# Fable3/CarND-Path-Planning-Project

Hardware: NVIDIA B200
Metric: planned frames/sec at 1M-frame batch (higher is better)
Workload: dtype f64

## Files before the change

### carnd-path-planning-project_b200/__init__.py

```python
from __future__ import annotations

import ctypes as C
import os

os.environ.setdefault("CUDA_DEVICE_MAX_CONNECTIONS", "32")

import numpy as np

from . import abi
from .abi import (Config, FrameBatch, Frames, PlanBatch, Plans, default_config, FLAG, FLAG_NAMES,
                  NUM_FLAGS, STATS_LEN, PATH_LEN, PREV_KEEP, MAP_STRIDE, FSTATS_LEN, FSTAT_NMIN,
                  FSTAT_NAMES, COMM_ID_BYTES)

_HERE = os.path.dirname(os.path.abspath(__file__))
LIB_PATH = os.path.join(_HERE, "libpp_b200.so")
ROOT = os.path.dirname(_HERE)
MAP_CSV = os.path.join(ROOT, "data", "highway_map.csv")

EXPORTS = [
    "pp_version", "pp_init", "pp_strerror", "pp_last_cuda_error", "pp_device_count", "pp_config_default",
    "pp_map_create", "pp_map_create_from_csv", "pp_map_destroy", "pp_map_num_waypoints",
    "pp_map_table", "pp_plan_batch", "pp_plan_batch_host", "pp_plan_batch_host_split", "pp_stats_batch",
    "pp_set_kernel_variant", "pp_launch_count", "pp_distancesq_pt_seg_batch",
    "pp_init_reference_waypoint_batch", "pp_lane_matching_batch", "pp_get_lane_pos_batch",
    "pp_spline_batch", "pp_closest_waypoint_batch", "pp_next_waypoint_batch",
    "pp_get_frenet_batch", "pp_get_xy_batch", "pp_synth_frames", "pp_selftest_math",
    "pp_lane_change_batch", "pp_limit_speed_batch", "pp_trajectory_build_batch",
    "pp_set_phase_timing", "pp_get_phase_ms", "pp_speed_controller_batch",
    "pp_project_speed_batch", "pp_control_points_batch",
    "pp_dev_alloc", "pp_dev_free", "pp_host_alloc", "pp_host_free", "pp_dev_upload", "pp_dev_download", "pp_dev_sync",
    "pp_dev_set", "pp_stream_create", "pp_stream_sync", "pp_stream_destroy",
    "pp_rollouts_create", "pp_rollouts_destroy", "pp_rollouts_run", "pp_rollouts_last",
    "pp_rollouts_get_state", "pp_rollouts_stats", "pp_rollouts_set_lean", "pp_rollouts_set_groups",
    "pp_rollouts_get_incidents", "pp_rollouts_incident_totals", "pp_rollouts_set_traffic",
    "pp_rollouts_get_traffic", "pp_rollouts_set_recorder", "pp_rollouts_get_recording",
    "pp_rollouts_set_surrogate", "pp_rollouts_get_surrogate", "pp_rollouts_surrogate_totals",
    "pp_sweep_batch",
    "pp_set_pipes", "pp_plan_stats_batch", "pp_synth_frames_dev", "pp_fstats_batch",
    "pp_comm_unique_id", "pp_comm_init_rank", "pp_comm_init_all", "pp_comm_destroy",
    "pp_comm_group_begin", "pp_comm_group_end", "pp_stats_reduce",
]


class PPError(RuntimeError):
    pass
# ... 511 lines not shown
```

### carnd-path-planning-project_b200/csrc/pp_api.cu

```cuda
#include <cuda_runtime.h>

#include <atomic>
#include <cstdint>
#include <cstdio>
#include <cstdlib>
#include <cstring>
#include <mutex>
#include <string>
#include <vector>

#include "pp_internal.h"

extern "C" int pp_init(void) {
  if (setenv("CUDA_DEVICE_MAX_CONNECTIONS", "32", 0) != 0) return PP_E_ARG;
  return PP_OK;
}

namespace {
std::mutex g_err_mu;
std::string g_err = "";
std::atomic<long long> g_launches{0};
}

namespace ppi {
// ... 11 lines not shown
int check_map_device(const pp_map *map, const char *who) {
  if (!map) return PP_E_ARG;
  if (!map->dev_table) {
    set_cuda_error(who, 0, "map has no device table (no usable CUDA device)");
    return PP_E_CUDA;
  }
  int dev = -1;
  cudaError_t e = cudaGetDevice(&dev);
  if (e != cudaSuccess) {
    set_cuda_error("cudaGetDevice", (int)e, cudaGetErrorString(e));
    cudaGetLastError();
    return PP_E_CUDA;
  }
  if (dev != map->device) {
    char msg[160];
    std::snprintf(msg, sizeof msg, "map lives on device %d but device %d is current", map->device,
                  dev);
    set_cuda_error(who, 0, msg);
    return PP_E_ARG;
  }
  return PP_OK;
}

int upload_map(pp_map *m) {
  int dev = 0;
  cudaError_t e = cudaGetDevice(&dev);
  if (e != cudaSuccess) {
    set_cuda_error("cudaGetDevice", (int)e, cudaGetErrorString(e));
    cudaGetLastError();
    return PP_E_CUDA;
  }
  const int pad = 24;
  static_assert(pad == PPD_PAD_ROWS, "padding must match the device code");
  std::vector<double> padded((size_t)(m->n + 2 * pad) * PP_MAP_STRIDE);
  for (int r = 0; r < m->n + 2 * pad; r++) {
    int src = (r - pad) % m->n;
    if (src < 0) src += m->n;
    std::memcpy(&padded[(size_t)r * PP_MAP_STRIDE], &m->table[(size_t)src * PP_MAP_STRIDE],
                PP_MAP_STRIDE * sizeof(double));
  }
  padded.resize(padded.size() + 2, 0.0);
  const size_t bytes = padded.size() * sizeof(double);
  e = cudaMalloc(&m->dev_table, bytes);
  if (e != cudaSuccess) {
    m->dev_table = nullptr;
    set_cuda_error("cudaMalloc(map)", (int)e, cudaGetErrorString(e));
    cudaGetLastError();
    return PP_E_CUDA;
  }
  e = cudaMemcpy(m->dev_table, padded.data(), bytes, cudaMemcpyHostToDevice);
  if (e != cudaSuccess) {
    cudaFree(m->dev_table);
    m->dev_table = nullptr;
    set_cuda_error("cudaMemcpy(map)", (int)e, cudaGetErrorString(e));
    cudaGetLastError();
    return PP_E_CUDA;
  }
  e = cudaMalloc(&m->dev_yaw, m->yaw.size() * sizeof(double));
  if (e == cudaSuccess)
    e = cudaMemcpy(m->dev_yaw, m->yaw.data(), m->yaw.size() * sizeof(double), cudaMemcpyHostToDevice);
  if (e != cudaSuccess) {
    cudaFree(m->dev_table);
// ... 91 lines not shown

int pp_map_create_from_csv(const char *path, pp_map **out) {
  if (!out) return PP_E_ARG;
  *out = nullptr;
  std::vector<double> wx, wy;
  int rc = ppi::read_map_csv(path, wx, wy);
  if (rc != PP_OK) return rc;
  return pp_map_create(wx.data(), wy.data(), (int)wx.size(), out);
}

void pp_map_destroy(pp_map *map) {
  if (!map) return;
  ppi::free_map_device(map);
  delete map;
}

int pp_map_num_waypoints(const pp_map *map) { return map ? map->n : PP_E_ARG; }

int pp_map_has_device(const pp_map *map) { return map && map->dev_table ? 1 : 0; }

int pp_map_table(const pp_map *map, double *out) {
  if (!map || !out) return PP_E_ARG;
  std::memcpy(out, map->table.data(), map->table.size() * sizeof(double));
  return PP_OK;
}

#define PP_CK(call, what)                                           \
  do {                                                              \
    cudaError_t e_ = (call);                                        \
    if (e_ != cudaSuccess) {                                        \
      ppi::set_cuda_error(what, (int)e_, cudaGetErrorString(e_));   \
      cudaGetLastError();                                           \
      return PP_E_CUDA;                                             \
    }                                                               \
  } while (0)

int pp_dev_alloc(void **out, size_t bytes) {
  if (!out) return PP_E_ARG;
  *out = nullptr;
  PP_CK(cudaMalloc(out, bytes ? bytes : 1), "pp_dev_alloc");
  return PP_OK;
}
int pp_dev_free(void *p) {
  if (p) PP_CK(cudaFree(p), "pp_dev_free");
  return PP_OK;
}
// ... 487 lines not shown
```

### carnd-path-planning-project_b200/csrc/pp_device.cuh

```cuda
#pragma once
#include <cstdint>

#include "../../include/pp.h"

namespace ppd {

#define PPD_EPS 1e-5
#define PPD_PI 3.14159265358979323846

#define PPD_INLINE __device__ __forceinline__

#define PPD_PAD 24
struct MapView {
  const double *t;
  int n;
  int pad_lo;
};

static __device__ __noinline__ int wrap_index(int idx, int n) {
  if (idx >= 0) return idx % n;
  idx += n;
  if (idx >= 0) return idx;
  unsigned long long k = (unsigned long long)(long long)idx;
  return (int)(k % (unsigned long long)n);
}

PPD_INLINE const double *row(const MapView &m, int idx) {
  if ((unsigned)(idx + m.pad_lo) < (unsigned)(m.n + m.pad_lo + PPD_PAD))
    return m.t + idx * PP_MAP_STRIDE;
  return m.t + wrap_index(idx, m.n) * PP_MAP_STRIDE;
}

__host__ __device__ inline size_t map_smem_doubles(int n) { return (size_t)(n + 2 * PPD_PAD) * PP_MAP_STRIDE; }

__host__ __device__ inline size_t map_stage_bytes(int n) {
  return (map_smem_doubles(n) * sizeof(double) + 15) & ~(size_t)15;
}

PPD_INLINE unsigned smem_addr(const void *p) { return (unsigned)__cvta_generic_to_shared(p); }
PPD_INLINE void mbar_init(unsigned bar, int count) {
  asm volatile("mbarrier.init.shared::cta.b64 [%0], %1;" ::"r"(bar), "r"(count) : "memory");
  asm volatile("fence.mbarrier_init.release.cluster;" ::: "memory");
}
PPD_INLINE void mbar_expect_tx(unsigned bar, unsigned bytes) {
  asm volatile("mbarrier.arrive.expect_tx.shared::cta.b64 _, [%0], %1;" ::"r"(bar), "r"(bytes)
               : "memory");
}
PPD_INLINE bool mbar_try_wait(unsigned bar, unsigned parity) {
  unsigned ok;
  asm volatile(
      "{\n"
      ".reg .pred p;\n"
      "mbarrier.try_wait.parity.shared::cta.b64 p, [%1], %2;\n"
      "selp.u32 %0, 1, 0, p;\n"
      "}\n"
      : "=r"(ok)
// ... 36 lines not shown
    asm volatile("mbarrier.init.shared::cta.b64 [%0], %1;" ::"r"(bar), "r"(1) : "memory");
    asm volatile("fence.mbarrier_init.release.cluster;" ::: "memory");
  }
  __syncthreads();
  if (threadIdx.x == 0) {
    asm volatile("mbarrier.arrive.expect_tx.shared::cta.b64 _, [%0], %1;" ::"r"(bar), "r"(bytes)
                 : "memory");
    asm volatile(
        "cp.async.bulk.shared::cluster.global.mbarrier::complete_tx::bytes [%0], [%1], %2, [%3];"
        ::"r"(dst), "l"(table), "r"(bytes), "r"(bar)
        : "memory");
  }
  asm volatile(
      "{\n"
      ".reg .pred p;\n"
      "WAIT_MAP:\n"
      "mbarrier.try_wait.parity.shared::cta.b64 p, [%0], %1;\n"
      "@p bra DONE_MAP;\n"
      "bra WAIT_MAP;\n"
      "DONE_MAP:\n"
      "}\n" ::"r"(bar), "r"(0)
      : "memory");
  MapView m;
  m.t = s_map + PPD_PAD * PP_MAP_STRIDE;
  m.n = n;
  m.pad_lo = n < PPD_PAD ? n : PPD_PAD;
  return m;
}

PPD_INLINE double vlen(double x, double y) { return sqrt(x * x + y * y); }
PPD_INLINE double dist4(double x1, double y1, double x2, double y2) {
  return sqrt((x2 - x1) * (x2 - x1) + (y2 - y1) * (y2 - y1));
}
PPD_INLINE double smax(double a, double b) { return (a < b) ? b : a; }
PPD_INLINE double smin(double a, double b) { return (b < a) ? b : a; }

PPD_INLINE bool safe_mag(double a) {
  const unsigned e = (unsigned)__double2hiint(a) & 0x7ff00000u;
  return e - ((1023u - 464u) << 20) < (928u << 20);
}
PPD_INLINE double div_rcp(double a, double b, double y) {
  const double q0 = a * y;
  const double r0 = fma(-b, q0, a);
  const double q1 = fma(r0, y, q0);
  const double r1 = fma(-b, q1, a);
  return fma(r1, y, q1);
}
// ... 109 lines not shown
    e = fma(e, s4, kAtanSeries[k]);
    o = fma(o, s4, kAtanSeries[k + 1]);
  }
  const double pl = fma(o, s2, e);
  double phi = base + fma(tq * s2, pl, tq);
  if (swap) phi = PPD_PI / 2 - phi;
  if (dx < 0) phi = PPD_PI - phi;
  return dy < 0 ? -phi : phi;
}
PPD_INLINE double wrap_lean(double x) {
  const double m = 2 * PPD_PI;
  const double t1 = x - m, t2 = x - 2 * m;
  const double t3 = t2 - m;
  const double hi = t2 < m ? t2 : t3;
  return x < m ? x : (x < 2 * m ? t1 : hi);
}

PPD_INLINE double lane_center_offset(int lane) { return 4.0 * (lane + 0.5); }

struct SegDist {
  double d2, rnom, rdenom, snom;
};

PPD_INLINE SegDist pt_seg(double px, double py, double ax, double ay, double bx, double by) {
  SegDist r;
  r.rnom = 0;
  r.rdenom = 1;
  r.snom = 0;
  if (ax == bx && ay == by) {
    r.d2 = (ax - bx) * (ax - bx) + (ay - by) * (ay - by);
    return r;
  }
  const double rdenom = (ax - bx) * (ax - bx) + (ay - by) * (ay - by);
  const double pdx = px - ax, dx = bx - ax;
  const double pdy = py - ay, dy = by - ay;
  const double rnom = pdx * dx + pdy * dy;
  const double snom = pdx * dy - pdy * dx;
  r.rdenom = rdenom;
  r.snom = snom;
  if (rnom < -1) {
    r.rnom = 0;
    r.d2 = (px - ax) * (px - ax) + (py - ay) * (py - ay);
    return r;
  }
  if (rnom > rdenom) {
    r.rnom = rdenom;
    r.d2 = (px - bx) * (px - bx) + (py - by) * (py - by);
    return r;
  }
  r.rnom = rnom;
  r.d2 = snom * snom / rdenom;
  return r;
}

PPD_INLINE double seg_ratio(double rnom, double rdenom) {
  if (rnom == 0) return rnom;
  if (rnom == rdenom && rdenom < 1e300) return 1.0;
  return rnom / rdenom;
}

struct RefState {
  int wp;
  double ratio[3];
};

PPD_INLINE void finish_reference(const MapView &m, double x, double y, int closest, RefState &rs) {
  const double *pr = row(m, closest - 1);
  const double *cr = row(m, closest);
  const double *nr = row(m, closest + 1);
  const SegDist s0 = pt_seg(x, y, pr[0], pr[1], cr[0], cr[1]);
  const SegDist s1 = pt_seg(x, y, cr[0], cr[1], nr[0], nr[1]);
  if (s1.d2 < s0.d2) {
    closest++;
  } else if (s1.d2 == s0.d2) {
    const double ax = (pr[8] + cr[8]) / 2;
    const double ay = (pr[9] + cr[9]) / 2;
    const double dpx = x - cr[0], dpy = y - cr[1];
    const double dotp = ax * dpx + ay * dpy;
    if (dotp > 0) closest++;
  }
  rs.wp = closest;
  const double *a = row(m, closest - 1);
  const double *b = row(m, closest);
#pragma unroll
  for (int lane = 0; lane < 3; lane++) {
    const SegDist s = pt_seg(x, y, a[2 + 2 * lane], a[3 + 2 * lane], b[2 + 2 * lane], b[3 + 2 * lane]);
    rs.ratio[lane] = seg_ratio(s.rnom, s.rdenom);
  }
}

PPD_INLINE void init_reference(const MapView &m, double x, double y, RefState &rs) {
  int closest = 0;
  double best = (m.t[0] - x) * (m.t[0] - x) + (m.t[1] - y) * (m.t[1] - y);
  for (int i = 1; i < m.n; i++) {
    const double rx = m.t[i * PP_MAP_STRIDE], ry = m.t[i * PP_MAP_STRIDE + 1];
    const double d = (rx - x) * (rx - x) + (ry - y) * (ry - y);
    if (d < best) {
      closest = i;
      best = d;
    }
  }
  finish_reference(m, x, y, closest, rs);
}

struct Match {
  bool ok;
  int lane, wp;
  double s, d;
};

struct WalkBest {
  bool ok;
  int lane, wp;
  double d2, rnom, rdenom, snom;
  double sum_s, s_ratio, seg_len;
};

PPD_INLINE void seg_rows(const MapView &m, int cur, const double *&a, const double *&b) {
  if ((unsigned)(cur - 1 + m.pad_lo) < (unsigned)(m.n + m.pad_lo + PPD_PAD - 1)) {
    a = m.t + (cur - 1) * PP_MAP_STRIDE;
    b = a + PP_MAP_STRIDE;
  } else {
    a = row(m, cur - 1);
    b = row(m, cur);
  }
}

struct SegRaw {
  double d2, rnom, rdenom, snom;
  int cls;
};
PPD_INLINE SegRaw seg_raw(double px, double py, double ax, double ay, double bx, double by) {
  SegRaw r;
  const double rdenom = (ax - bx) * (ax - bx) + (ay - by) * (ay - by);
  const double pdx = px - ax, dx = bx - ax;
  const double pdy = py - ay, dy = by - ay;
  const double rnom = pdx * dx + pdy * dy;
  r.snom = pdx * dy - pdy * dx;
  r.rdenom = rdenom;
  r.rnom = rnom;
  r.d2 = 0;
  r.cls = 2;
  if (ax == bx && ay == by) {
    r.cls = 3;
    r.rnom = 0;
    r.rdenom = 1;
    r.snom = 0;
    r.d2 = rdenom;
  } else if (rnom < -1) {
    r.cls = 0;
    r.rnom = 0;
    r.d2 = pdx * pdx + pdy * pdy;
  } else if (rnom > rdenom) {
    r.cls = 1;
    r.rnom = rdenom;
    r.d2 = (px - bx) * (px - bx) + (py - by) * (py - by);
  }
  return r;
}

PPD_INLINE WalkBest lane_walk(const MapView &m, const RefState &rs, double x, double y) {
  const unsigned mask = __activemask();
  int dir = 0;
  bool stop = false;
  int cur = rs.wp;
  double best = 1000 * 1000;
  int b_code = -1;
  int steps = 0;
  int step_dir = 1;
  bool done = false;
  for (;;) {
    const double *a = m.t, *b = m.t;
    if (!done) {
      for (;;) {
        seg_rows(m, cur, a, b);
        double d2[3];
        unsigned fwd = 0;
        bool interior = false;
#pragma unroll
        for (int lane = 0; lane < 3; lane++) {
          const double ax = a[2 + 2 * lane], ay = a[3 + 2 * lane];
          const double bx = b[2 + 2 * lane], by = b[3 + 2 * lane];
          const double dx = bx - ax, dy = by - ay;
          const double rdenom = dx * dx + dy * dy;
          const double pdx = x - ax, pdy = y - ay;
          const double rnom = pdx * dx + pdy * dy;
          const bool deg = (dx == 0) & (dy == 0);
          const bool to_a = rnom < -1;
          const bool to_b = !to_a & (rnom > rdenom);
          interior |= !deg & !to_a & !to_b;
          const double qx = to_b ? x - bx : pdx, qy = to_b ? y - by : pdy;
          const double dq = qx * qx + qy * qy;
          d2[lane] = deg ? rdenom : dq;
          fwd |= (unsigned)(!deg & to_b & (rdenom != 0)) << lane;
        }
        if (interior) break;
        bool improved = false;
#pragma unroll
        for (int lane = 0; lane < 3; lane++) {
          if (d2[lane] < best) {
            best = d2[lane];
            improved = true;
            b_code = (steps << 2) | lane;
          }
        }
        {
          const unsigned mix = (fwd ^ (fwd >> 1)) & 3u;
          const int d0 = (fwd & 1u) ? 1 : -1;
          stop |= (mix != 0u) | ((dir != 0) & (dir != d0));
          dir = (fwd & 4u) ? 1 : -1;
        }
        if (!improved | stop) {
          done = true;
          break;
        }
        step_dir = dir;
        cur += dir;
        steps++;
      }
    }
    if (!__any_sync(mask, !done)) break;
    if (!done) {
      bool improved = false;
#pragma unroll
      for (int lane = 0; lane < 3; lane++) {
        const SegDist sd =
            pt_seg(x, y, a[2 + 2 * lane], a[3 + 2 * lane], b[2 + 2 * lane], b[3 + 2 * lane]);
        if (sd.d2 < best) {
          best = sd.d2;
          improved = true;
          b_code = (steps << 2) | lane;
        }
        if (sd.rnom == 0) {
          if (dir == 1) stop = true;
          dir = -1;
        } else if (sd.rnom == sd.rdenom) {
          if (dir == -1) stop = true;
          dir = 1;
        } else {
          stop = true;
        }
      }
      if (!improved || stop) {
        done = true;
      } else {
        step_dir = dir > 0 ? 1 : -1;
        cur += step_dir;
        steps++;
      }
    }
  }

  WalkBest w;
  w.ok = b_code >= 0;
  w.lane = 0;
  w.wp = 0;
  w.d2 = 0;
  w.rnom = 0;
  w.rdenom = 1;
  w.snom = 0;
  w.sum_s = 0;
  w.s_ratio = 0;
  w.seg_len = 0;
  if (w.ok) {
    const int b_lane = b_code & 3, b_steps = b_code >> 2;
    const int sdir = step_dir;
    double sum = 0;
    double ratio = b_lane == 0 ? rs.ratio[0] : (b_lane == 1 ? rs.ratio[1] : rs.ratio[2]);
    int wp = rs.wp;
    for (int k = 0; k < b_steps; k++) {
      const double len = row(m, wp)[10 + b_lane];
      if (sdir > 0) {
        sum += (1 - ratio) * len;
        ratio = 0;
        wp++;
      } else {
        sum -= ratio * len;
        ratio = 1;
        wp--;
      }
    }
    const double *a, *b;
    seg_rows(m, wp, a, b);
    const SegRaw q = seg_raw(x, y, a[2 + 2 * b_lane], a[3 + 2 * b_lane], b[2 + 2 * b_lane],
                             b[3 + 2 * b_lane]);
    w.lane = b_lane;
    w.wp = wp;
    w.d2 = best;
    w.rnom = q.rnom;
    w.rdenom = q.rdenom;
    w.snom = q.snom;
    w.sum_s = sum;
    w.s_ratio = ratio;
    w.seg_len = b[10 + b_lane];
  }
  return w;
}

PPD_INLINE Match finish_match(const WalkBest &w) {
  Match r;
  r.ok = w.ok;
  r.lane = w.lane;
  r.wp = w.wp;
  r.s = 0;
  r.d = 0;
  if (w.ok) {
    const double from_start = seg_ratio(w.rnom, w.rdenom);
    const double r_mod = from_start - w.s_ratio;
    r.s = w.sum_s + w.seg_len * r_mod;
    double d = sqrt(w.d2);
    if (w.snom < 0) d = -d;
    r.d = d + lane_center_offset(w.lane);
  }
  return r;
}

PPD_INLINE Match lane_match(const MapView &m, const RefState &rs, double x, double y) {
  return finish_match(lane_walk(m, rs, x, y));
}

PPD_INLINE void project_speed(const MapView &m, double vx, double vy, int next_wp, double &vs,
                              double &vd) {
  const double vl = vlen(vx, vy);
  if (vl < PPD_EPS) {
    vs = vl;
    vd = 0;
    return;
  }
  const double *a = row(m, next_wp);
  const double *b = row(m, next_wp - 1);
// ... 1256 lines not shown
```

### carnd-path-planning-project_b200/csrc/pp_internal.h

```cpp
#pragma once
#include <cstdint>
#include <vector>

#include "../../include/pp.h"

#define PPD_PAD_ROWS 24

struct pp_map {
  int n = 0;
  std::vector<double> table;
  double *dev_table = nullptr;
  int device = -1;
  std::vector<double> yaw;
  double *dev_yaw = nullptr;
};

namespace ppi {

int build_map_table(const double *wx, const double *wy, int n, std::vector<double> &table);
void build_yaw_table(const std::vector<double> &table, int n, std::vector<double> &yaw);
int read_map_csv(const char *path, std::vector<double> &wx, std::vector<double> &wy);

int upload_map(pp_map *m);
void free_map_device(pp_map *m);

void set_cuda_error(const char *what, int cuda_err, const char *text);
int check_map_device(const pp_map *map, const char *who);

size_t plan_scratch_bytes(int64_t n_frames, int max_cars);
// ... 69 lines not shown
```

### carnd-path-planning-project_b200/csrc/pp_plan.cu

```cuda
#include <cuda.h>
#include <cuda_runtime.h>

#include <atomic>
#include <cstdio>
#include <cstdlib>
#include <cstring>
#include <mutex>
#include <vector>

#include "pp_device.cuh"
#include "pp_internal.h"

namespace {

using namespace ppd;

constexpr int kBlock = 128;
#ifndef PP_PREP_MINB
#define PP_PREP_MINB 5
#endif
#ifndef PP_CARS_MINB
#define PP_CARS_MINB 6
#endif
#ifndef PP_DECIDE_MINB
#define PP_DECIDE_MINB 4
#endif

struct FrameCtx {
  double x, y, speed, acc;
  int nprev;
  RefState rs;
  int lane;
  double s, d, vs, vd;
  uint32_t flags;
// ... 282 lines not shown
PPD_INLINE void plan_one_frame(const MapView &m, const pp_config &cfg, const pp_frames &in,
                               const pp_plans &out, int64_t f) {
  const FrameCtx c = stage_prep(m, cfg, in, f);
  uint32_t flags = c.flags;
  const int mc = in.max_cars;
  int nc = in.n_cars[f];
  if (nc > mc) nc = mc;
  const int tl_in = in.target_lane_in[f];
  Behav b;
  behav_init(b, cfg);
  const int64_t cb = f * mc;
  for (int j = 0; j < nc; j++) {
    const CarRes r = car_slot(m, c.rs, in, cb + j, in.car_x[cb + j], in.car_y[cb + j],
                              in.car_vx[cb + j], in.car_vy[cb + j]);
    store_car(out, cb + j, r);
    behav_add(b, cfg, c, tl_in, in.car_id[cb + j], j, r, flags);
  }
  stage_finish(m, cfg, in, out, f, c, b, tl_in, flags);
}

PPD_INLINE int warp_closest_waypoint(const MapView &m, double x, double y) {
  const int lane = threadIdx.x & 31;
  int closest = lane < m.n ? lane : 0;
  double best = (m.t[closest * PP_MAP_STRIDE] - x) * (m.t[closest * PP_MAP_STRIDE] - x) +
                (m.t[closest * PP_MAP_STRIDE + 1] - y) * (m.t[closest * PP_MAP_STRIDE + 1] - y);
  for (int i = lane + 32; i < m.n; i += 32) {
    const double rx = m.t[i * PP_MAP_STRIDE], ry = m.t[i * PP_MAP_STRIDE + 1];
    const double d = (rx - x) * (rx - x) + (ry - y) * (ry - y);
    if (d < best) {
      closest = i;
      best = d;
    }
  }
#pragma unroll
  for (int o = 1; o < 32; o <<= 1) {
    const double od = __shfl_xor_sync(0xffffffffu, best, o);
    const int oi = __shfl_xor_sync(0xffffffffu, closest, o);
    if (od < best || (od == best && oi < closest)) {
      best = od;
      closest = oi;
    }
  }
  return __shfl_sync(0xffffffffu, closest, 0);
}

PPD_INLINE void plan_one_frame_warp(const MapView &m, const pp_config &cfg, const pp_frames &in,
                                    const pp_plans &out, int64_t f) {
  const int lane = threadIdx.x & 31;
  FrameCtx c;
  double svx, svy;
// ... 704 lines not shown
      for (int o = 1; o < G; o <<= 1) behav_merge_xor(bp, pflags, o);
      if (act && k == 0) behav_store(sc, f, bp, pflags);
    }
    fence_async_smem();
    __syncwarp();
  }
}

template <bool kBehav>
__global__ void __launch_bounds__(kBlock, PP_DECIDE_MINB)
k_decide_t(const double *__restrict__ map_table, int n_wp, const __grid_constant__ pp_config cfg,
           const __grid_constant__ pp_frames in, const __grid_constant__ pp_plans out,
           const __grid_constant__ Scratch sc, int64_t n, int bulk_in, int bulk_out,
           const __grid_constant__ CUtensorMap tm_x, const __grid_constant__ CUtensorMap tm_y) {
  extern __shared__ __align__(128) double s_dyn[];
  double *s_rows = s_dyn;
  double *s_px = s_dyn + PPD_SWEEP_ROWS * PPD_TAILK * kBlock;
  double *s_py = s_px + kBlock * PP_PREV_KEEP;
  __shared__ __align__(8) unsigned long long s_bar;
  const unsigned bar = smem_addr(&s_bar);
  if (threadIdx.x == 0) mbar_init(bar, 1);
  __syncthreads();
  MapView m;
  m.t = map_table + PPD_PAD * PP_MAP_STRIDE;
  m.n = n_wp;
  m.pad_lo = n_wp < PPD_PAD ? n_wp : PPD_PAD;
  const int64_t n_tiles = (n + kBlock - 1) / kBlock;
  long long xacc = 0;
  unsigned phase = 0;
  for (int64_t tile = blockIdx.x; tile < n_tiles; tile += gridDim.x) {
    const int64_t f0 = tile * kBlock;
    const int nf = (int)((n - f0) < kBlock ? (n - f0) : kBlock);
    const unsigned bytes = (unsigned)nf * PP_PREV_KEEP * 8u;
    if (bulk_in && threadIdx.x == 0) {
      mbar_expect_tx(bar, 2u * bytes);
      bulk_g2s(smem_addr(s_px), in.prev_x + f0 * PP_PREV_KEEP, bytes, bar);
      bulk_g2s(smem_addr(s_py), in.prev_y + f0 * PP_PREV_KEEP, bytes, bar);
    }
    const int64_t f = f0 + threadIdx.x;
    const bool own = threadIdx.x < nf;
    FrameCtx c;
    Decision d;
    if (own) {
      load_ctx(sc, f, c);
      uint32_t flags = c.flags;
      const int tl_in = in.target_lane_in[f];
      Behav b;
// ... 864 lines not shown
```

### carnd-path-planning-project_b200/csrc/pp_rollout.cu

```cuda
#include <cuda_runtime.h>

#include <cmath>
#include <cstdio>
#include <cstdlib>
#include <cstring>
#include <utility>
#include <vector>

#include "pp_device.cuh"
#include "pp_internal.h"

struct pp_rollouts {
  const pp_map *map = nullptr;
  int64_t n = 0;
  int32_t c = 0;
  uint64_t seed = 0;
  int64_t first = 0;
  int64_t tick = 0;
  char *buf = nullptr;
  double *ego_x, *ego_y, *ego_yaw, *ego_mph, *car_ratio, *car_speed;
  int32_t *path_n, *path_off, *target_lane, *car_lane, *car_wp;
  bool lean = false;
  pp_plans full_pl;
  pp_frames fr;
// ... 1076 lines not shown
Traffic traffic_view(const pp_rollouts *r) {
  return Traffic{r->trf_v0, r->trf_acc, r->trf_cum, r->trf_ego_lanes, r->trf_ego_s,
                 r->fr.ego_speed_mph, r->n};
}

Recorder recorder_view(const pp_rollouts *r) {
  return Recorder{r->rec_ring, r->rec_trig_tick, r->rec_trig_bits, r->n, r->c, r->rec_w, r->rec_mask};
}

Surrogate surrogate_view(const pp_rollouts *r) {
  return Surrogate{r->ssm_min, r->ssm_tick, r->ssm_hist, r->n};
}

template <int kTraffic>
auto advance_kernel(bool rec, bool ssm) {
  return rec ? (ssm ? k_sim_advance<kTraffic, true, true> : k_sim_advance<kTraffic, true, false>)
             : (ssm ? k_sim_advance<kTraffic, false, true> : k_sim_advance<kTraffic, false, false>);
}

size_t traffic_smem_bytes(int c) { return (size_t)c * kR * (8 + 8 + 4); }

int issue_tick(pp_rollouts *r, const pp_config *cfg, int32_t consume_k, cudaStream_t st,
               bool fork = true, bool join = true) {
  const Track trk{r->map->dev_table + (size_t)PPD_PAD_ROWS * PP_MAP_STRIDE, r->map->n, PP_MAP_STRIDE};
  static const int forced_groups = [] {
    const char *e = getenv("PP_ROLLOUT_GROUPS");
    const int v = e && *e ? atoi(e) : 0;
    return v < 0 ? 0 : (v > pp_rollouts::kGroups ? pp_rollouts::kGroups : v);
  }();
  const int forced = r->groups_wanted ? r->groups_wanted : forced_groups;
  int groups = forced ? forced : pp_rollouts::kGroups;
  while (groups > 1 && r->n / groups < (forced ? 4096 : 16384)) groups--;
  const int64_t per = (r->n + groups - 1) / groups;
  const int mc = r->fr.max_cars;
  if (fork) {
    cudaEventRecord(r->fork, st);
    for (int g = 0; g < groups; g++) cudaStreamWaitEvent(r->gs[g], r->fork, 0);
  }
  const int64_t launches0 = pp_launch_count();
  for (int g = 0; g < groups; g++) {
    const int64_t lo = g * per;
    const int64_t cnt = (r->n - lo) < per ? (r->n - lo) : per;
    if (cnt <= 0) continue;
    cudaStream_t gs = r->gs[g];
    const int grid = (int)((cnt + kR - 1) / kR);
    const pp_frames fr = ppi::offset_frames(r->fr, lo);
    const pp_plans pl = ppi::offset_plans(r->pl, lo, mc);
// ... 225 lines not shown
    r->trf_cum = (double *)b;
    b += al(3 * (size_t)(nw + 1) * 8);
    r->trf_ego_lanes = (int32_t *)b;
    b += al(2 * N * 4);
    r->trf_ego_s = (double *)b;
  }
  std::vector<double> cum(3 * (size_t)(nw + 1));
  for (int L = 0; L < 3; L++) {
    double acc = 0.0;
    cum[(size_t)L * (nw + 1)] = 0.0;
    for (int w = 0; w < nw; w++) {
      acc += r->map->table[(size_t)w * PP_MAP_STRIDE + 10 + L];
      cum[(size_t)L * (nw + 1) + w + 1] = acc;
    }
  }
  cudaError_t e = cudaMemcpy(r->trf_cum, cum.data(), cum.size() * 8, cudaMemcpyHostToDevice);
  if (e == cudaSuccess && NC)
    e = cudaMemcpy(r->trf_v0, r->car_speed, NC * 8, cudaMemcpyDeviceToDevice);
  if (e == cudaSuccess && NC) e = cudaMemset(r->trf_acc, 0, NC * 8);
  if (e != cudaSuccess) {
    r->traffic = PP_TRAFFIC_CONSTANT;
    return cuda_fail("pp_rollouts_set_traffic", e);
  }
  const Track trk{r->map->dev_table + (size_t)PPD_PAD_ROWS * PP_MAP_STRIDE, nw, PP_MAP_STRIDE};
  k_traffic_init<<<(int)((r->n + kB - 1) / kB), kB>>>(trk, r->ego_x, r->ego_y, traffic_view(r));
  ppi::count_launch(1);
  e = cudaDeviceSynchronize();
  if (e == cudaSuccess) e = cudaGetLastError();
  if (e != cudaSuccess) {
    r->traffic = PP_TRAFFIC_CONSTANT;
    return cuda_fail("k_traffic_init", e);
  }
  return PP_OK;
}

extern "C" int pp_rollouts_get_traffic(const pp_rollouts *r, pp_rollout_traffic *h) {
  if (!r || !h || r->traffic != PP_TRAFFIC_IDM) return PP_E_ARG;
  cudaError_t e = cudaDeviceSynchronize();
  if (e != cudaSuccess) return cuda_fail("pp_rollouts_get_traffic", e);
  const size_t N = (size_t)r->n, NC = (size_t)r->n * (size_t)r->c;
  const int buf = (int)(r->tick & 1);
  bool ok = true;
  auto dn = [&](void *dst, const void *src, size_t bytes) {
    if (dst && bytes && cudaMemcpy(dst, src, bytes, cudaMemcpyDeviceToHost) != cudaSuccess) ok = false;
  };
  dn(h->car_v0, r->trf_v0, NC * 8);
  dn(h->car_acc, r->trf_acc, NC * 8);
// ... 247 lines not shown
```

### carnd-path-planning-project_b200/csrc/pp_sweep.cu

```cuda
#include <cuda_runtime.h>

#include <cstdio>

#include "pp_device.cuh"
#include "pp_internal.h"

namespace {

using namespace ppd;

constexpr int kCandPerLane = PP_SWEEP_SPEEDS * PP_SWEEP_TIMES;
constexpr int kHead = 7;
constexpr int kRows = kHead + 5 * PPD_TAILK;

struct SweepScratch {
  double *est;
  int32_t *np;
  int32_t *code;
  double *scores;
  int64_t n3;
};

PPD_INLINE void ego_pose(const pp_frames &in, int64_t f, double &x, double &y, int &nprev) {
  if (in.prev_n[f] >= PP_PREV_KEEP) {
    x = in.prev_x[f * PP_PREV_KEEP + PP_PREV_KEEP - 1];
    y = in.prev_y[f * PP_PREV_KEEP + PP_PREV_KEEP - 1];
    nprev = PP_PREV_KEEP;
  } else {
    x = in.ego_x[f];
    y = in.ego_y[f];
    nprev = 0;
  }
}

__global__ void __launch_bounds__(128)
k_sweep_setup(const double *__restrict__ map_table, int n_wp, const __grid_constant__ pp_config cfg,
              const __grid_constant__ pp_frames in, const double *__restrict__ ego_d,
              const double *__restrict__ ego_vd, const double *__restrict__ ego_speed,
              const __grid_constant__ SweepScratch sw, int64_t n) {
  extern __shared__ __align__(16) double s_rows[];
  MapView m;
  m.t = map_table + PPD_PAD * PP_MAP_STRIDE;
  m.n = n_wp;
  m.pad_lo = n_wp < PPD_PAD ? n_wp : PPD_PAD;
  const int64_t q = (int64_t)blockIdx.x * blockDim.x + threadIdx.x;
  if (q >= 3 * n) return;
  const int64_t f = q / 3;
  const int lane = (int)(q - f * 3);
  double x, y;
  int nprev;
  ego_pose(in, f, x, y, nprev);
  RefState rs;
  init_reference(m, x, y, rs);
  SpeedCtl sc;
  sc_init(sc, cfg, ego_speed[f]);
  double kept_x[PP_PREV_KEEP], kept_y[PP_PREV_KEEP];
  uint32_t flags = 0;
  double *e = sw.est + q;
  KnotSweep ks;
  ks.init(s_rows + threadIdx.x, blockDim.x, e, sw.n3, kHead);
  TrajFrame tf;
  traj_setup(m, cfg, rs, in.prev_x + f * PP_PREV_KEEP, in.prev_y + f * PP_PREV_KEEP, nprev, x, y,
             in.ego_yaw_deg[f], lane, ego_d[f], ego_vd[f], sc, kept_x, kept_y, flags, ks, tf);
  e[0 * sw.n3] = sc.start;
  e[3 * sw.n3] = tf.cx;
// ... 243 lines not shown
```

### carnd-path-planning-project_b200/csrc/pp_synth.cu

```cuda
#include <cuda_runtime.h>

#include <cmath>
#include <cstdint>

#include "pp_internal.h"

#define PP_HD __host__ __device__

namespace {

template <class T>
PP_HD inline void swap2(T &a, T &b) {
  const T t = a;
  a = b;
  b = t;
}

struct Rng {
  uint64_t key, ctr;
  PP_HD static uint64_t mix(uint64_t z) {
    z += 0x9E3779B97F4A7C15ull;
    z = (z ^ (z >> 30)) * 0xBF58476D1CE4E5B9ull;
    z = (z ^ (z >> 27)) * 0x94D049BB133111EBull;
    return z ^ (z >> 31);
  }
  PP_HD Rng(uint64_t seed, uint64_t frame) : key(mix(mix(seed) ^ (frame * 0xD1B54A32D192ED03ull))), ctr(0) {}
  PP_HD uint64_t next() { return mix(key + (ctr++) * 0x9E3779B97F4A7C15ull); }
  PP_HD double uni() { return (double)(next() >> 11) * (1.0 / 9007199254740992.0); }
  PP_HD double range(double a, double b) { return a + (b - a) * uni(); }
  PP_HD int below(int n) { return (int)(next() % (uint64_t)n); }
  PP_HD bool chance(double p) { return uni() < p; }
};

struct Track {
  const double *t;
  const double *yaw;
  int n;
  PP_HD int wrap(int i) const { return ((i % n) + n) % n; }
  PP_HD const double *row(int i) const { return t + (size_t)(((i % n) + n) % n) * PP_MAP_STRIDE; }
  PP_HD void at(int w, double u, int lane, double &x, double &y, double &tx, double &ty, double &nx,
          double &ny) const {
    const double *a = row(w - 1), *b = row(w);
    const double ax = a[2 + 2 * lane], ay = a[3 + 2 * lane];
    const double bx = b[2 + 2 * lane], by = b[3 + 2 * lane];
    const double len = b[10 + lane];
    x = ax + (bx - ax) * u;
    y = ay + (by - ay) * u;
    tx = (bx - ax) / len;
    ty = (by - ay) / len;
    nx = b[8];
    ny = b[9];
  }
  PP_HD void walk(int &w, double &u, int lane, double ds) const {
    for (int guard = 0; guard < 4 * n; guard++) {
      const double len = row(w)[10 + lane];
      if (ds >= 0) {
        const double rem = len * (1 - u);
        if (ds <= rem) {
          u += ds / len;
          return;
        }
        ds -= rem;
// ... 161 lines not shown
}

}

void ppi::build_yaw_table(const std::vector<double> &table, int n, std::vector<double> &yaw) {
  yaw.assign((size_t)n * PP_NUM_LANES, 0.0);
  for (int w = 0; w < n; w++) {
    const double *a = &table[(size_t)((w - 1 + n) % n) * PP_MAP_STRIDE];
    const double *b = &table[(size_t)w * PP_MAP_STRIDE];
    for (int lane = 0; lane < PP_NUM_LANES; lane++) {
      const double len = b[10 + lane];
      const double tx = (b[2 + 2 * lane] - a[2 + 2 * lane]) / len;
      const double ty = (b[3 + 2 * lane] - a[3 + 2 * lane]) / len;
      yaw[(size_t)w * PP_NUM_LANES + lane] = std::atan2(ty, tx) * 180 / M_PI;
    }
  }
}

extern "C" int pp_synth_frames(const pp_map *map, uint64_t seed, int64_t first_frame,
                               int64_t n_frames, int32_t n_cars, int32_t rare_permille,
                               const pp_frames *out) {
  const int rc = check_out(map, n_frames, n_cars, out);
  if (rc != PP_OK) return rc;
  Track trk{map->table.data(), map->yaw.data(), map->n};
  for (int64_t f = 0; f < n_frames; f++)
    synth_one(trk, seed, first_frame + f, n_cars, rare_permille, out, f);
  return PP_OK;
}

extern "C" int pp_synth_frames_dev(const pp_map *map, uint64_t seed, int64_t first_frame,
                                   int64_t n_frames, int32_t n_cars, int32_t rare_permille,
                                   const pp_frames *out_dev, void *cuda_stream) {
  int rc = check_out(map, n_frames, n_cars, out_dev);
  if (rc != PP_OK) return rc;
  if ((rc = ppi::check_map_device(map, "pp_synth_frames_dev")) != PP_OK) return rc;
  if (n_frames == 0) return PP_OK;
  Track trk{map->dev_table + (size_t)PPD_PAD_ROWS * PP_MAP_STRIDE, map->dev_yaw, map->n};
  const int64_t want = (n_frames + 127) / 128;
  const int grid = (int)(want < 148 * 16 ? want : 148 * 16);
  k_synth<<<grid, 128, 0, (cudaStream_t)cuda_stream>>>(trk, seed, first_frame, n_frames, n_cars,
                                                      rare_permille, *out_dev);
  ppi::count_launch();
  cudaError_t e = cudaGetLastError();
  if (e != cudaSuccess) {
    ppi::set_cuda_error("k_synth", (int)e, cudaGetErrorString(e));
    return PP_E_CUDA;
  }
  return PP_OK;
}
```

### include/pp.h

```cpp
#ifndef PP_B200_H
#define PP_B200_H

#include <stddef.h>
#include <stdint.h>

#ifdef __cplusplus
extern "C" {
#endif

#define PP_VERSION 102

#define PP_NUM_LANES 3
#define PP_PREV_KEEP 10
#define PP_PATH_LEN 50
#define PP_MAX_CARS 64

#define PP_MAP_STRIDE 13

#define PP_OK 0
#define PP_E_ARG (-1)
#define PP_E_CUDA (-2)
#define PP_E_IO (-3)
#define PP_E_NOMEM (-4)
#define PP_E_RANGE (-5)
// ... 80 lines not shown

#define PP_STAT_FRAMES 0
#define PP_STAT_POINTS 1
#define PP_STAT_TARGET_LANE0 2
#define PP_STAT_EGO_LANE0 5
#define PP_STAT_LANE_CHANGES 8
#define PP_STAT_FLAG0 9
#define PP_STAT_XSUM (PP_STAT_FLAG0 + PP_NUM_FLAGS)
#define PP_STATS_LEN (PP_STAT_XSUM + 1)

int pp_version(void);
int pp_init(void);
const char *pp_strerror(int code);
const char *pp_last_cuda_error(void);
int pp_device_count(void);

int pp_config_default(pp_config *cfg);

int pp_map_create(const double *wx, const double *wy, int n, pp_map **out);
int pp_map_create_from_csv(const char *path, pp_map **out);
void pp_map_destroy(pp_map *map);
int pp_map_num_waypoints(const pp_map *map);
int pp_map_table(const pp_map *map, double *out);

int pp_plan_batch(const pp_map *map, const pp_config *cfg, const pp_frames *in,
                  const pp_plans *out, int64_t n_frames, void *cuda_stream);

int pp_plan_batch_host(const pp_map *map, const pp_config *cfg, const pp_frames *in,
                       const pp_plans *out, int64_t n_frames);

typedef struct pp_split_rows {
  double *head_x, *head_y;
  double *tail_x, *tail_y;
} pp_split_rows;
int pp_plan_batch_host_split(const pp_map *map, const pp_config *cfg, const pp_frames *in,
                             const pp_plans *out, const pp_split_rows *rows, int64_t n_frames);

int pp_stats_batch(const pp_plans *plans_dev, int64_t n_frames, int64_t *stats_dev,
                   void *cuda_stream);

#define PP_FSTAT_MIN_EGO_SPEED 0
#define PP_FSTAT_MIN_TARGET_SPEED 1
#define PP_FSTAT_MIN_STEP_SPEED 2
#define PP_FSTAT_NMIN 3
#define PP_FSTAT_MAX_EGO_SPEED 3
#define PP_FSTAT_MAX_TARGET_SPEED 4
// ... 241 lines not shown
```

Before: 416.7 million.

## Widen map rows with precomputed segment reciprocals and add clamped lane walk

Extends each padded device map row from 13 to 18 doubles. The new columns hold host-precomputed reciprocals of the per-lane segment length squared, plus a validity bitmask, so point-to-segment divisions become multiplies when the reciprocal is safe. The lane walk gains a tight clamped inner loop that keeps stepping in one direction without the warp-wide control logic, and lane points are loaded as double2 pairs. The wider rows raise shared-memory staging size and may lower occupancy, and every consumer of the table has to use the new stride.

```diff
diff --git a/carnd-path-planning-project_b200/__init__.py b/carnd-path-planning-project_b200/__init__.py
--- a/carnd-path-planning-project_b200/__init__.py
+++ b/carnd-path-planning-project_b200/__init__.py
@@ -20,7 +20,7 @@
 EXPORTS = [
     "pp_version", "pp_init", "pp_strerror", "pp_last_cuda_error", "pp_device_count", "pp_config_default",
     "pp_map_create", "pp_map_create_from_csv", "pp_map_destroy", "pp_map_num_waypoints",
-    "pp_map_table", "pp_plan_batch", "pp_plan_batch_host", "pp_plan_batch_host_split", "pp_stats_batch",
+    "pp_map_table", "pp_map_device_table", "pp_plan_batch", "pp_plan_batch_host", "pp_plan_batch_host_split", "pp_stats_batch",
     "pp_set_kernel_variant", "pp_launch_count", "pp_distancesq_pt_seg_batch",
     "pp_init_reference_waypoint_batch", "pp_lane_matching_batch", "pp_get_lane_pos_batch",
     "pp_spline_batch", "pp_closest_waypoint_batch", "pp_next_waypoint_batch",
diff --git a/carnd-path-planning-project_b200/csrc/pp_api.cu b/carnd-path-planning-project_b200/csrc/pp_api.cu
--- a/carnd-path-planning-project_b200/csrc/pp_api.cu
+++ b/carnd-path-planning-project_b200/csrc/pp_api.cu
@@ -57,6 +57,13 @@
   return PP_OK;
 }
 
+static bool rcp_usable(double b) {
+  uint64_t bits;
+  std::memcpy(&bits, &b, sizeof bits);
+  const unsigned e = (unsigned)(bits >> 52) & 0x7ffu;
+  return e - (1023u - 464u) < 928u && (bits & 0xFFFFFFFFFFFFFull) != 0xFFFFFFFFFFFFFull;
+}
+
 int upload_map(pp_map *m) {
   int dev = 0;
   cudaError_t e = cudaGetDevice(&dev);
@@ -67,12 +74,24 @@
   }
   const int pad = 24;
   static_assert(pad == PPD_PAD_ROWS, "padding must match the device code");
-  std::vector<double> padded((size_t)(m->n + 2 * pad) * PP_MAP_STRIDE);
+  const int w = PPD_STRIDE_COLS;
+  std::vector<double> padded((size_t)(m->n + 2 * pad) * w, 0.0);
   for (int r = 0; r < m->n + 2 * pad; r++) {
     int src = (r - pad) % m->n;
     if (src < 0) src += m->n;
-    std::memcpy(&padded[(size_t)r * PP_MAP_STRIDE], &m->table[(size_t)src * PP_MAP_STRIDE],
-                PP_MAP_STRIDE * sizeof(double));
+    const double *b = &m->table[(size_t)src * PP_MAP_STRIDE];
+    const double *a = &m->table[(size_t)((src + m->n - 1) % m->n) * PP_MAP_STRIDE];
+    double *d = &padded[(size_t)r * w];
+    std::memcpy(d, b, PP_MAP_STRIDE * sizeof(double));
+    uint64_t ok = 0;
+    for (int lane = 0; lane < 3; lane++) {
+      const double ax = a[2 + 2 * lane], ay = a[3 + 2 * lane];
+      const double bx = b[2 + 2 * lane], by = b[3 + 2 * lane];
+      const double rdenom = (ax - bx) * (ax - bx) + (ay - by) * (ay - by);
+      d[13 + lane] = 1.0 / rdenom;
+      ok |= (uint64_t)rcp_usable(rdenom) << lane;
+    }
+    std::memcpy(&d[16], &ok, sizeof ok);
   }
   padded.resize(padded.size() + 2, 0.0);
   const size_t bytes = padded.size() * sizeof(double);
@@ -210,6 +229,23 @@
 int pp_map_table(const pp_map *map, double *out) {
   if (!map || !out) return PP_E_ARG;
   std::memcpy(out, map->table.data(), map->table.size() * sizeof(double));
+  return PP_OK;
+}
+
+int pp_map_device_table(const pp_map *map, double *out, int32_t *stride, int32_t *pad) {
+  if (!map) return PP_E_ARG;
+  if (stride) *stride = PPD_STRIDE_COLS;
+  if (pad) *pad = PPD_PAD_ROWS;
+  if (!out) return PP_OK;
+  int rc = ppi::check_map_device(map, "pp_map_device_table");
+  if (rc != PP_OK) return rc;
+  const size_t bytes = (size_t)(map->n + 2 * PPD_PAD_ROWS) * PPD_STRIDE_COLS * sizeof(double);
+  cudaError_t e = cudaMemcpy(out, map->dev_table, bytes, cudaMemcpyDeviceToHost);
+  if (e != cudaSuccess) {
+    ppi::set_cuda_error("cudaMemcpy(map)", (int)e, cudaGetErrorString(e));
+    cudaGetLastError();
+    return PP_E_CUDA;
+  }
   return PP_OK;
 }
 
diff --git a/carnd-path-planning-project_b200/csrc/pp_device.cuh b/carnd-path-planning-project_b200/csrc/pp_device.cuh
--- a/carnd-path-planning-project_b200/csrc/pp_device.cuh
+++ b/carnd-path-planning-project_b200/csrc/pp_device.cuh
@@ -11,6 +11,9 @@
 #define PPD_INLINE __device__ __forceinline__
 
 #define PPD_PAD 24
+#define PPD_STRIDE 18
+#define PPD_COL_RCP 13
+#define PPD_COL_RCP_OK 16
 struct MapView {
   const double *t;
   int n;
@@ -27,11 +30,11 @@
 
 PPD_INLINE const double *row(const MapView &m, int idx) {
   if ((unsigned)(idx + m.pad_lo) < (unsigned)(m.n + m.pad_lo + PPD_PAD))
-    return m.t + idx * PP_MAP_STRIDE;
-  return m.t + wrap_index(idx, m.n) * PP_MAP_STRIDE;
-}
-
-__host__ __device__ inline size_t map_smem_doubles(int n) { return (size_t)(n + 2 * PPD_PAD) * PP_MAP_STRIDE; }
+    return m.t + idx * PPD_STRIDE;
+  return m.t + wrap_index(idx, m.n) * PPD_STRIDE;
+}
+
+__host__ __device__ inline size_t map_smem_doubles(int n) { return (size_t)(n + 2 * PPD_PAD) * PPD_STRIDE; }
 
 __host__ __device__ inline size_t map_stage_bytes(int n) {
   return (map_smem_doubles(n) * sizeof(double) + 15) & ~(size_t)15;
@@ -114,7 +117,7 @@
       "}\n" ::"r"(bar), "r"(0)
       : "memory");
   MapView m;
-  m.t = s_map + PPD_PAD * PP_MAP_STRIDE;
+  m.t = s_map + PPD_PAD * PPD_STRIDE;
   m.n = n;
   m.pad_lo = n < PPD_PAD ? n : PPD_PAD;
   return m;
@@ -270,7 +273,27 @@
   double d2, rnom, rdenom, snom;
 };
 
-PPD_INLINE SegDist pt_seg(double px, double py, double ax, double ay, double bx, double by) {
+struct SegRcp {
+  double y;
+  bool ok;
+};
+PPD_INLINE SegRcp seg_rcp(const double *a, const double *b, int lane) {
+  SegRcp r;
+  r.y = b[PPD_COL_RCP + lane];
+  r.ok = (b == a + PPD_STRIDE) &
+         ((((unsigned)__double2loint(b[PPD_COL_RCP_OK]) >> lane) & 1u) != 0u);
+  return r;
+}
+PPD_INLINE Rcp with_rcp(double rdenom, const SegRcp &sr) {
+  Rcp r;
+  r.b = rdenom;
+  r.y = sr.y;
+  r.ok = sr.ok;
+  return r;
+}
+
+PPD_INLINE SegDist pt_seg(double px, double py, double ax, double ay, double bx, double by,
+                          const SegRcp &sr) {
   SegDist r;
   r.rnom = 0;
   r.rdenom = 1;
@@ -297,14 +320,20 @@
     return r;
   }
   r.rnom = rnom;
-  r.d2 = snom * snom / rdenom;
+  r.d2 = div_by(snom * snom, with_rcp(rdenom, sr));
   return r;
 }
-
-PPD_INLINE double seg_ratio(double rnom, double rdenom) {
+PPD_INLINE SegDist pt_seg(double px, double py, double ax, double ay, double bx, double by) {
+  SegRcp none;
+  none.y = 0;
+  none.ok = false;
+  return pt_seg(px, py, ax, ay, bx, by, none);
+}
+
+PPD_INLINE double seg_ratio(double rnom, double rdenom, const SegRcp &sr) {
   if (rnom == 0) return rnom;
   if (rnom == rdenom && rdenom < 1e300) return 1.0;
-  return rnom / rdenom;
+  return div_by(rnom, with_rcp(rdenom, sr));
 }
 
 struct RefState {
@@ -332,8 +361,10 @@
   const double *b = row(m, closest);
 #pragma unroll
   for (int lane = 0; lane < 3; lane++) {
-    const SegDist s = pt_seg(x, y, a[2 + 2 * lane], a[3 + 2 * lane], b[2 + 2 * lane], b[3 + 2 * lane]);
-    rs.ratio[lane] = seg_ratio(s.rnom, s.rdenom);
+    const SegRcp sr = seg_rcp(a, b, lane);
+    const SegDist s =
+        pt_seg(x, y, a[2 + 2 * lane], a[3 + 2 * lane], b[2 + 2 * lane], b[3 + 2 * lane], sr);
+    rs.ratio[lane] = seg_ratio(s.rnom, s.rdenom, sr);
   }
 }
 
@@ -341,7 +372,7 @@
   int closest = 0;
   double best = (m.t[0] - x) * (m.t[0] - x) + (m.t[1] - y) * (m.t[1] - y);
   for (int i = 1; i < m.n; i++) {
-    const double rx = m.t[i * PP_MAP_STRIDE], ry = m.t[i * PP_MAP_STRIDE + 1];
+    const double rx = m.t[i * PPD_STRIDE], ry = m.t[i * PPD_STRIDE + 1];
     const double d = (rx - x) * (rx - x) + (ry - y) * (ry - y);
     if (d < best) {
       closest = i;
@@ -362,12 +393,20 @@
   int lane, wp;
   double d2, rnom, rdenom, snom;
   double sum_s, s_ratio, seg_len;
+  SegRcp rcp;
 };
 
+PPD_INLINE bool seg_in_window(const MapView &m, int cur) {
+  return (unsigned)(cur - 1 + m.pad_lo) < (unsigned)(m.n + m.pad_lo + PPD_PAD - 1);
+}
+PPD_INLINE double2 lane_pt(const double *r, int lane) {
+  return *reinterpret_cast<const double2 *>(r + 2 + 2 * lane);
+}
+
 PPD_INLINE void seg_rows(const MapView &m, int cur, const double *&a, const double *&b) {
-  if ((unsigned)(cur - 1 + m.pad_lo) < (unsigned)(m.n + m.pad_lo + PPD_PAD - 1)) {
-    a = m.t + (cur - 1) * PP_MAP_STRIDE;
-    b = a + PP_MAP_STRIDE;
+  if (seg_in_window(m, cur)) {
+    a = m.t + (cur - 1) * PPD_STRIDE;
+    b = a + PPD_STRIDE;
   } else {
     a = row(m, cur - 1);
     b = row(m, cur);
@@ -407,6 +446,47 @@
   return r;
 }
 
+PPD_INLINE bool take_best(const double (&d2)[3], int steps, double &best, int &b_code) {
+  bool improved = false;
+#pragma unroll
+  for (int lane = 0; lane < 3; lane++) {
+    if (d2[lane] < best) {
+      best = d2[lane];
+      improved = true;
+      b_code = (steps << 2) | lane;
+    }
+  }
+  return improved;
+}
+
+PPD_INLINE bool walk_clamped(const MapView &m, double x, double y, int dir, int &cur, int &steps,
+                             double &best, int &b_code) {
+  const bool fwd = dir > 0;
+  for (;;) {
+    if (!seg_in_window(m, cur)) return false;
+    const double *a = m.t + (cur - 1) * PPD_STRIDE;
+    const double *b = a + PPD_STRIDE;
+    const double *e = fwd ? b : a;
+    bool all = true;
+    double d2[3];
+#pragma unroll
+    for (int lane = 0; lane < 3; lane++) {
+      const double2 pa = lane_pt(a, lane), pb = lane_pt(b, lane), pe = lane_pt(e, lane);
+      const double dx = pb.x - pa.x, dy = pb.y - pa.y;
+      const double rdenom = dx * dx + dy * dy;
+      const double pdx = x - pa.x, pdy = y - pa.y;
+      const double rnom = pdx * dx + pdy * dy;
+      all &= fwd ? (rnom > rdenom) & (rdenom != 0) : rnom < -1;
+      const double qx = x - pe.x, qy = y - pe.y;
+      d2[lane] = qx * qx + qy * qy;
+    }
+    if (!all) return false;
+    if (!take_best(d2, steps, best, b_code)) return true;
+    cur += dir;
+    steps++;
+  }
+}
+
 PPD_INLINE WalkBest lane_walk(const MapView &m, const RefState &rs, double x, double y) {
   const unsigned mask = __activemask();
   int dir = 0;
@@ -427,8 +507,8 @@
         bool interior = false;
 #pragma unroll
         for (int lane = 0; lane < 3; lane++) {
-          const double ax = a[2 + 2 * lane], ay = a[3 + 2 * lane];
-          const double bx = b[2 + 2 * lane], by = b[3 + 2 * lane];
+          const double2 pa = lane_pt(a, lane), pb = lane_pt(b, lane);
+          const double ax = pa.x, ay = pa.y, bx = pb.x, by = pb.y;
           const double dx = bx - ax, dy = by - ay;
           const double rdenom = dx * dx + dy * dy;
           const double pdx = x - ax, pdy = y - ay;
@@ -443,15 +523,7 @@
           fwd |= (unsigned)(!deg & to_b & (rdenom != 0)) << lane;
         }
         if (interior) break;
-        bool improved = false;
-#pragma unroll
-        for (int lane = 0; lane < 3; lane++) {
-          if (d2[lane] < best) {
-            best = d2[lane];
-            improved = true;
-            b_code = (steps << 2) | lane;
-          }
-        }
+        const bool improved = take_best(d2, steps, best, b_code);
         {
           const unsigned mix = (fwd ^ (fwd >> 1)) & 3u;
           const int d0 = (fwd & 1u) ? 1 : -1;
@@ -465,6 +537,12 @@
         step_dir = dir;
         cur += dir;
         steps++;
+        if (walk_clamped(m, x, y, dir, cur, steps, best, b_code)) {
+          done = true;
+          break;
+        }
+        seg_rows(m, cur, a, b);
+        break;
       }
     }
     if (!__any_sync(mask, !done)) break;
@@ -472,8 +550,8 @@
       bool improved = false;
 #pragma unroll
       for (int lane = 0; lane < 3; lane++) {
-        const SegDist sd =
-            pt_seg(x, y, a[2 + 2 * lane], a[3 + 2 * lane], b[2 + 2 * lane], b[3 + 2 * lane]);
+        const double2 pa = lane_pt(a, lane), pb = lane_pt(b, lane);
+        const SegDist sd = pt_seg(x, y, pa.x, pa.y, pb.x, pb.y, seg_rcp(a, b, lane));
         if (sd.d2 < best) {
           best = sd.d2;
           improved = true;
@@ -510,6 +588,8 @@
   w.sum_s = 0;
   w.s_ratio = 0;
   w.seg_len = 0;
+  w.rcp.y = 0;
+  w.rcp.ok = false;
   if (w.ok) {
     const int b_lane = b_code & 3, b_steps = b_code >> 2;
     const int sdir = step_dir;
@@ -541,6 +621,7 @@
     w.sum_s = sum;
     w.s_ratio = ratio;
     w.seg_len = b[10 + b_lane];
+    w.rcp = seg_rcp(a, b, b_lane);
   }
   return w;
 }
@@ -553,7 +634,7 @@
   r.s = 0;
   r.d = 0;
   if (w.ok) {
-    const double from_start = seg_ratio(w.rnom, w.rdenom);
+    const double from_start = seg_ratio(w.rnom, w.rdenom, w.rcp);
     const double r_mod = from_start - w.s_ratio;
     r.s = w.sum_s + w.seg_len * r_mod;
     double d = sqrt(w.d2);
diff --git a/carnd-path-planning-project_b200/csrc/pp_internal.h b/carnd-path-planning-project_b200/csrc/pp_internal.h
--- a/carnd-path-planning-project_b200/csrc/pp_internal.h
+++ b/carnd-path-planning-project_b200/csrc/pp_internal.h
@@ -5,6 +5,7 @@
 #include "../../include/pp.h"
 
 #define PPD_PAD_ROWS 24
+#define PPD_STRIDE_COLS 18
 
 struct pp_map {
   int n = 0;
diff --git a/carnd-path-planning-project_b200/csrc/pp_plan.cu b/carnd-path-planning-project_b200/csrc/pp_plan.cu
--- a/carnd-path-planning-project_b200/csrc/pp_plan.cu
+++ b/carnd-path-planning-project_b200/csrc/pp_plan.cu
@@ -10,6 +10,8 @@
 
 #include "pp_device.cuh"
 #include "pp_internal.h"
+
+static_assert(PPD_STRIDE == PPD_STRIDE_COLS, "device map rows must match upload_map");
 
 namespace {
 
@@ -338,10 +340,10 @@
 PPD_INLINE int warp_closest_waypoint(const MapView &m, double x, double y) {
   const int lane = threadIdx.x & 31;
   int closest = lane < m.n ? lane : 0;
-  double best = (m.t[closest * PP_MAP_STRIDE] - x) * (m.t[closest * PP_MAP_STRIDE] - x) +
-                (m.t[closest * PP_MAP_STRIDE + 1] - y) * (m.t[closest * PP_MAP_STRIDE + 1] - y);
+  double best = (m.t[closest * PPD_STRIDE] - x) * (m.t[closest * PPD_STRIDE] - x) +
+                (m.t[closest * PPD_STRIDE + 1] - y) * (m.t[closest * PPD_STRIDE + 1] - y);
   for (int i = lane + 32; i < m.n; i += 32) {
-    const double rx = m.t[i * PP_MAP_STRIDE], ry = m.t[i * PP_MAP_STRIDE + 1];
+    const double rx = m.t[i * PPD_STRIDE], ry = m.t[i * PPD_STRIDE + 1];
     const double d = (rx - x) * (rx - x) + (ry - y) * (ry - y);
     if (d < best) {
       closest = i;
@@ -1092,7 +1094,7 @@
   if (threadIdx.x == 0) mbar_init(bar, 1);
   __syncthreads();
   MapView m;
-  m.t = map_table + PPD_PAD * PP_MAP_STRIDE;
+  m.t = map_table + PPD_PAD * PPD_STRIDE;
   m.n = n_wp;
   m.pad_lo = n_wp < PPD_PAD ? n_wp : PPD_PAD;
   const int64_t n_tiles = (n + kBlock - 1) / kBlock;
diff --git a/carnd-path-planning-project_b200/csrc/pp_rollout.cu b/carnd-path-planning-project_b200/csrc/pp_rollout.cu
--- a/carnd-path-planning-project_b200/csrc/pp_rollout.cu
+++ b/carnd-path-planning-project_b200/csrc/pp_rollout.cu
@@ -1122,7 +1122,7 @@
 
 int issue_tick(pp_rollouts *r, const pp_config *cfg, int32_t consume_k, cudaStream_t st,
                bool fork = true, bool join = true) {
-  const Track trk{r->map->dev_table + (size_t)PPD_PAD_ROWS * PP_MAP_STRIDE, r->map->n, PP_MAP_STRIDE};
+  const Track trk{r->map->dev_table + (size_t)PPD_PAD_ROWS * PPD_STRIDE_COLS, r->map->n, PPD_STRIDE_COLS};
   static const int forced_groups = [] {
     const char *e = getenv("PP_ROLLOUT_GROUPS");
     const int v = e && *e ? atoi(e) : 0;
@@ -1394,7 +1394,7 @@
     r->traffic = PP_TRAFFIC_CONSTANT;
     return cuda_fail("pp_rollouts_set_traffic", e);
   }
-  const Track trk{r->map->dev_table + (size_t)PPD_PAD_ROWS * PP_MAP_STRIDE, nw, PP_MAP_STRIDE};
+  const Track trk{r->map->dev_table + (size_t)PPD_PAD_ROWS * PPD_STRIDE_COLS, nw, PPD_STRIDE_COLS};
   k_traffic_init<<<(int)((r->n + kB - 1) / kB), kB>>>(trk, r->ego_x, r->ego_y, traffic_view(r));
   ppi::count_launch(1);
   e = cudaDeviceSynchronize();
diff --git a/carnd-path-planning-project_b200/csrc/pp_sweep.cu b/carnd-path-planning-project_b200/csrc/pp_sweep.cu
--- a/carnd-path-planning-project_b200/csrc/pp_sweep.cu
+++ b/carnd-path-planning-project_b200/csrc/pp_sweep.cu
@@ -40,7 +40,7 @@
               const __grid_constant__ SweepScratch sw, int64_t n) {
   extern __shared__ __align__(16) double s_rows[];
   MapView m;
-  m.t = map_table + PPD_PAD * PP_MAP_STRIDE;
+  m.t = map_table + PPD_PAD * PPD_STRIDE;
   m.n = n_wp;
   m.pad_lo = n_wp < PPD_PAD ? n_wp : PPD_PAD;
   const int64_t q = (int64_t)blockIdx.x * blockDim.x + threadIdx.x;
diff --git a/carnd-path-planning-project_b200/csrc/pp_synth.cu b/carnd-path-planning-project_b200/csrc/pp_synth.cu
--- a/carnd-path-planning-project_b200/csrc/pp_synth.cu
+++ b/carnd-path-planning-project_b200/csrc/pp_synth.cu
@@ -36,8 +36,9 @@
   const double *t;
   const double *yaw;
   int n;
+  int stride;
   PP_HD int wrap(int i) const { return ((i % n) + n) % n; }
-  PP_HD const double *row(int i) const { return t + (size_t)(((i % n) + n) % n) * PP_MAP_STRIDE; }
+  PP_HD const double *row(int i) const { return t + (size_t)(((i % n) + n) % n) * stride; }
   PP_HD void at(int w, double u, int lane, double &x, double &y, double &tx, double &ty, double &nx,
           double &ny) const {
     const double *a = row(w - 1), *b = row(w);
@@ -245,7 +246,7 @@
                                const pp_frames *out) {
   const int rc = check_out(map, n_frames, n_cars, out);
   if (rc != PP_OK) return rc;
-  Track trk{map->table.data(), map->yaw.data(), map->n};
+  Track trk{map->table.data(), map->yaw.data(), map->n, PP_MAP_STRIDE};
   for (int64_t f = 0; f < n_frames; f++)
     synth_one(trk, seed, first_frame + f, n_cars, rare_permille, out, f);
   return PP_OK;
@@ -258,7 +259,8 @@
   if (rc != PP_OK) return rc;
   if ((rc = ppi::check_map_device(map, "pp_synth_frames_dev")) != PP_OK) return rc;
   if (n_frames == 0) return PP_OK;
-  Track trk{map->dev_table + (size_t)PPD_PAD_ROWS * PP_MAP_STRIDE, map->dev_yaw, map->n};
+  Track trk{map->dev_table + (size_t)PPD_PAD_ROWS * PPD_STRIDE_COLS, map->dev_yaw, map->n,
+            PPD_STRIDE_COLS};
   const int64_t want = (n_frames + 127) / 128;
   const int grid = (int)(want < 148 * 16 ? want : 148 * 16);
   k_synth<<<grid, 128, 0, (cudaStream_t)cuda_stream>>>(trk, seed, first_frame, n_frames, n_cars,
diff --git a/include/pp.h b/include/pp.h
--- a/include/pp.h
+++ b/include/pp.h
@@ -126,6 +126,7 @@
 void pp_map_destroy(pp_map *map);
 int pp_map_num_waypoints(const pp_map *map);
 int pp_map_table(const pp_map *map, double *out);
+int pp_map_device_table(const pp_map *map, double *out, int32_t *stride, int32_t *pad);
 
 int pp_plan_batch(const pp_map *map, const pp_config *cfg, const pp_frames *in,
                   const pp_plans *out, int64_t n_frames, void *cuda_stream);
diff --git a/profiles/sass_by_line.py b/profiles/sass_by_line.py
--- /dev/null
+++ b/profiles/sass_by_line.py
@@ -0,0 +1,38 @@
+import re
+import subprocess
+import sys
+
+
+def main():
+    cubin, kern, ranges = sys.argv[1], sys.argv[2], sys.argv[3:]
+    out = subprocess.run(["/usr/local/cuda/bin/nvdisasm", "-c", "-g", cubin], capture_output=True,
+                         text=True, check=True).stdout
+    funcs = re.split(r"\n\s*\.text\.", out)
+    body = next(f for f in funcs[1:] if kern in f.split("\n", 1)[0])
+    loc = None
+    counts = {r: {"all": 0, "LDS.128": 0, "LDS.64": 0, "FP64": 0} for r in ranges}
+    for line in body.split("\n"):
+        m = re.search(r'## File "([^"]+)", line (\d+)', line)
+        if m:
+            loc = (m.group(1).rsplit("/", 1)[-1], int(m.group(2)))
+            continue
+        m = re.search(r"/\*[0-9a-f]{4,}\*/\s+(?:@!?U?P\w+\s+)?([A-Z][A-Z0-9_.]*)", line)
+        if not m or loc is None:
+            continue
+        op = m.group(1)
+        for r in ranges:
+            f, span = r.split(":")
+            lo, hi = (int(v) for v in span.split("-"))
+            if loc[0] == f and lo <= loc[1] <= hi:
+                c = counts[r]
+                c["all"] += 1
+                c["LDS.128"] += op.startswith("LDS.128")
+                c["LDS.64"] += op.startswith("LDS.64")
+                c["FP64"] += op.split(".")[0] in ("DADD", "DMUL", "DFMA", "DSETP")
+    for r, c in counts.items():
+        print(f"{r}: {c['all']} instructions, LDS.128 {c['LDS.128']}, LDS.64 {c['LDS.64']}, "
+              f"FP64 {c['FP64']}")
+
+
+if __name__ == "__main__":
+    main()
```

Result: no change. 412.9 million (median of 6 runs) (-0.9%).
